# uguryagmur/RealTimeObjectDetection

Measured on AMD Instinct MI355X. Metric: frames/sec YOLOv3 608x608 bs=8 (Darknet.forward + write_results; 2 batches in flight, write_results_async on a second stream), higher is better.
Workload: dtype f16x2-split (3 MFMA products, f32 accumulate); 1 GPU; YOLOv3 cfg 608x608 batch=8 per GPU, split-f16 MFMA conv + fused head + GPU NMS (BASELINE configs[2]); precision=f16s3, tiles=autotune (this run), parallelism=frame-shard x1, in_flight_batches=2, detections_last_step=1699, candidates_last_step=1914, f16_range_overflow=False

## Files before the change

### realtimeobjectdetection_amd/csrc/capi.cpp

```cpp
#include <cstring>
#include <new>

#include "plan.h"

namespace rtod { const std::string& last_error_string(); }
using namespace rtod;

struct rtod_plan { Plan p; };

#define RTOD_GUARD_BEGIN try {
#define RTOD_GUARD_END                                                                   \
    } catch (const std::bad_alloc&) { set_error("out of host memory"); return RTOD_E_ARG; } \
      catch (const std::exception& e) { set_error("internal error: %s", e.what()); return RTOD_E_ARG; } \
      catch (...) { set_error("internal error"); return RTOD_E_ARG; }

extern "C" {

int rtod_version(void) { return 100; }

int rtod_last_error(char* buf, size_t len) {
    if (!buf || !len) return RTOD_E_ARG;
    const std::string& e = last_error_string();
    const size_t n = e.size() < len - 1 ? e.size() : len - 1;
    memcpy(buf, e.data(), n);
// ... 51 lines not shown
    memset(o, 0, sizeof(*o));
    o->n_layers = (int32_t)p.layers.size(); o->n_launches = (int32_t)p.launches.size();
    o->height = p.height; o->width = p.width; o->max_batch = p.max_batch;
    o->total_rows = p.total_rows; o->attrs = p.attrs;
    o->n_weight_floats = p.n_weight_floats; o->conv_flops_per_frame = p.conv_flops;
    o->arena_bytes = p.arena_floats * 4; o->packed_weight_bytes = p.packed_floats * 4;
    return RTOD_OK;
}

int rtod_plan_get_launch(const rtod_plan* plan, int index, rtod_launch_info* out) {
    if (!plan || !out || index < 0 || index >= (int)plan->p.launches.size()) { set_error("plan_get_launch: bad index"); return RTOD_E_ARG; }
    plan->p.fill_launch_info(index, out, plan->p.tuned.empty() ? plan->p.max_batch : plan->p.tuned.rbegin()->first);
    return RTOD_OK;
}

int rtod_plan_describe(const rtod_plan* plan, char* buf, size_t len, size_t* needed) {
    RTOD_GUARD_BEGIN
    if (!plan) { set_error("plan_describe: null plan"); return RTOD_E_ARG; }
    const std::string s = plan->p.describe();
    if (needed) *needed = s.size() + 1;
    if (buf && len) {
        const size_t n = s.size() < len - 1 ? s.size() : len - 1;
        memcpy(buf, s.data(), n);
        buf[n] = 0;
    }
    return RTOD_OK;
    RTOD_GUARD_END
}

const char* rtod_conv_variant_name(int variant) {
    if (variant == 100 + STEM2_VARIANT) return "conv_stem2_f16s3<2 x 4x16, stem + 3x3 s2 + 1x1>";
    if (variant >= 100 + PATCH_VARIANT_BASE && variant < 100 + PATCH_VARIANT_BASE + PATCH_MODES) return conv_patch_mode_info(variant - 100 - PATCH_VARIANT_BASE).name;
    if (variant >= 100 + PWD_VARIANT_BASE && variant < 100 + PWD_VARIANT_BASE + PWD_MODES) return conv_pwd_mode_info(variant - 100 - PWD_VARIANT_BASE).name;
    if (variant >= 100 + RING_VARIANT_BASE && variant < 100 + RING_VARIANT_BASE + RING_MODES) return conv_ring_mode_info(variant - 100 - RING_VARIANT_BASE).name;
    if (variant >= 100 + BAND_VARIANT_BASE && variant < 100 + BAND_VARIANT_BASE + BAND_MODES) return conv_band_mode_info(variant - 100 - BAND_VARIANT_BASE).name;
    if (variant >= 100 && variant < 100 + HV_COUNT) return conv_f16s3_variant_info(variant - 100).name;
    if (variant < 0 || variant % 10 >= CV_COUNT || variant / 10 > 2) return "";
    static const char* const kSliced[2][CV_COUNT] = {
        {"conv_igemm_f32<128x128,w64x64,k-slices>", "conv_igemm_f32<128x64,w64x32,k-slices>", "conv_igemm_f32<64x64,w32x32,k-slices>", "conv_igemm_f32<128x32,w32x32,k-slices>"},
        {"conv_igemm_f32<128x128,w64x64,wg per k-slice>", "conv_igemm_f32<128x64,w64x32,wg per k-slice>", "conv_igemm_f32<64x64,w32x32,wg per k-slice>", "conv_igemm_f32<128x32,w32x32,wg per k-slice>"}};
    if (variant >= 10) return kSliced[variant / 10 - 1][variant % 10];
    return conv_variant_info(variant).name;
}

int rtod_conv_kernel_name(int variant, int epilogue, char* buf, size_t len) {
    if (!buf || len == 0) { set_error("conv_kernel_name: null buffer"); return RTOD_E_ARG; }
    int n = -1;
    if (variant >= 100 + PATCH_VARIANT_BASE) n = conv_patch_kernel_name(variant - 100 - PATCH_VARIANT_BASE, epilogue, buf, len);
    else if (variant >= 100 + PWD_VARIANT_BASE) n = conv_pwd_kernel_name(variant - 100 - PWD_VARIANT_BASE, epilogue, buf, len);
    else if (variant >= 100 + RING_VARIANT_BASE) n = conv_ring_kernel_name(variant - 100 - RING_VARIANT_BASE, epilogue, buf, len);
    else if (variant >= 100 + BAND_VARIANT_BASE) n = conv_band_kernel_name(variant - 100 - BAND_VARIANT_BASE, epilogue, buf, len);
    else if (variant >= 100) n = conv_f16s3_kernel_name(variant - 100, epilogue, buf, len);
    else n = conv_f32_kernel_name(variant, buf, len);
    if (n < 0 || (size_t)n >= len) { set_error("conv_kernel_name: unknown variant %d or buffer too small", variant); return RTOD_E_ARG; }
    return RTOD_OK;
}

int rtod_plan_launch_kernel_name(const rtod_plan* plan, int index, char* buf, size_t len) {
    RTOD_GUARD_BEGIN
    if (!plan || !buf || len == 0 || index < 0 || index >= (int)plan->p.launches.size()) { set_error("launch_kernel_name: bad args"); return RTOD_E_ARG; }
    rtod_launch_info li;
    plan->p.fill_launch_info(index, &li, plan->p.tuned.empty() ? plan->p.max_batch : plan->p.tuned.rbegin()->first);
    buf[0] = 0;
    if (li.kind != LK_CONV || li.flops_per_frame == 0) return RTOD_OK;
    int epi = li.fused_decode ? 2 : (li.fused_pointwise ? (li.fused_residual ? 4 : 3) : (li.fused_residual ? 1 : 0));
    if (plan->p.precision == 2 && li.variant >= 100) epi |= EPI_F16;
    int n = -1;
    if (li.variant == 100 + STEM2_VARIANT) n = conv_stem2_kernel_name(li.fused_pointwise, buf, len);
    else return rtod_conv_kernel_name(li.variant, epi, buf, len);
    if (n < 0 || (size_t)n >= len) { set_error("launch_kernel_name: buffer too small"); return RTOD_E_ARG; }
    return RTOD_OK;
    RTOD_GUARD_END
}

int rtod_plan_set_precision(rtod_plan* plan, int mode) {
    if (!plan || mode < 0 || mode > 2) { set_error("set_precision: mode must be 0 (fp32), 1 (f16 split) or 2 (plain f16)"); return RTOD_E_ARG; }
    if (plan->p.d_weights) { set_error("set_precision: must be called before rtod_plan_load_weights"); return RTOD_E_STATE; }
    if (mode >= 1) { const int rc = plan->p.check_split_supported(mode); if (rc) return rc; }
    plan->p.precision = mode;
    plan->p.layout_weights();
    return RTOD_OK;
}
// ... 196 lines not shown
```

### realtimeobjectdetection_amd/csrc/plan.cpp

```cpp
#include "plan.h"

#include <algorithm>
#include <cctype>
#include <cmath>
#include <cstdarg>
#include <cstdlib>
#include <cstring>
#include <map>
#include <mutex>
#include <sstream>

namespace rtod {

static thread_local std::string g_err;

void set_error(const char* fmt, ...) {
    char buf[1024];
    va_list ap;
    va_start(ap, fmt);
    vsnprintf(buf, sizeof(buf), fmt, ap);
    va_end(ap);
    g_err = buf;
}
const std::string& last_error_string() { return g_err; }
// ... 240 lines not shown
            prev_is_decoded = true;
            pc = layers[i - 1].cout; ph = layers[i - 1].hout; pw = layers[i - 1].wout;
        } else {
            prev_is_decoded = false;
            pc = L.cout; ph = L.hout; pw = L.wout;
        }
        if (L.type == LT_ROUTE || L.type == LT_SHORTCUT) prev_is_decoded = false;
    }
    total_rows = row_off;
    n_weight_floats = woff;
    if (total_rows == 0) { set_error("cfg: no yolo layer (the reference would return [])"); return RTOD_E_CFG; }
    return RTOD_OK;
}

static int resolve_alias(const std::vector<Layer>& layers, int i) {
    while (layers[i].alias_of >= 0) i = layers[i].alias_of;
    return i;
}

void Plan::reset_planning() {
    for (auto& L : layers) { L.fused_into = -1; L.fused_away = false; L.buf = -1; L.coff = 0; L.alias_of = -1; }
    bufs.clear(); launches.clear(); convs.clear(); input_buf = -1;
    tuned.clear(); tune_cache.clear(); tuning.clear();
}

int Plan::set_option(const char* name, int value) {
    if (!name) { set_error("set_option: null name"); return RTOD_E_ARG; }
    if (d_weights) { set_error("set_option: must be called before rtod_plan_load_weights"); return RTOD_E_STATE; }
    const std::string k(name);
    bool* flag = nullptr; int* num = nullptr;
    if (k == "fuse_pointwise") flag = &opt_fuse_pointwise;
    else if (k == "ring_kernel") flag = &opt_ring_kernel;
    else if (k == "pwd_kernel") flag = &opt_pwd_kernel;
    else if (k == "stem2_kernel") flag = &opt_stem2_kernel;
    else if (k == "k_slices") flag = &opt_k_slices;
    else if (k == "bn_batch_stats") {
        if (value && height != width) { set_error("set_option: bn_batch_stats is not supported on a rectangular plan (%dx%d)", height, width); return RTOD_E_ARG; }
        flag = &opt_bn_batch_stats;
    }
    else if (k == "k_slice_workgroups") flag = &opt_k_slice_workgroups;
    else if (k == "patch_kernel") flag = &opt_patch_kernel;
    else if (k == "stem_kernel") flag = &opt_stem_kernel;
    else if (k == "band_kernel") flag = &opt_band_kernel;
    else if (k == "fuse_shortcut") flag = &opt_fuse_shortcut;
    else if (k == "fuse_decode") flag = &opt_fuse_decode;
    else if (k == "zero_copy_concat") flag = &opt_zero_copy_concat;
    else if (k == "force_f16s3_variant") num = &opt_force_f16s3_variant;
    else if (k == "force_f32_variant") num = &opt_force_f32_variant;
    else { set_error("set_option: unknown option '%s'", name); return RTOD_E_ARG; }
    const bool old_flag = flag ? *flag : false; const int old_num = num ? *num : 0;
    if (flag) *flag = value != 0; else *num = value;
    reset_planning();
    int rc = plan_buffers();
    if (!rc && precision >= 1) rc = check_split_supported(precision);
    if (rc) {
        const std::string msg = last_error_string();
        if (flag) *flag = old_flag; else *num = old_num;
        reset_planning();
        (void)plan_buffers();
        set_error("%s", msg.c_str());
    }
    return rc;
}

int Plan::plan_buffers() {
    const int n = (int)layers.size();
// ... 434 lines not shown
    const PackedConv& pc = convs[l.conv_slot];
    if (pc.split || pc.stem || pc.slice_chunks <= 0) return 0;
    const Layer& L = layers[l.layer];
    const ConvVariantInfo& vi = conv_variant_info(variant);
    const int64_t M = (int64_t)batch * L.hout * L.wout;
    const int64_t tiles = ((M + vi.bm - 1) / vi.bm) * ((L.cout + vi.bn - 1) / vi.bn);
    const int64_t S = (pc.Kpad / 32 + pc.slice_chunks - 1) / pc.slice_chunks;
    return (opt_k_slice_workgroups && d_scratch && tiles < 512 && S * M * pc.Npad <= scratch_floats) ? 2 : 1;
}

static bool variant_has_f16(int v) {
    return (v >= 0 && v < HV_COUNT) || (v >= BAND_VARIANT_BASE + BAND_LDS_MODES && v < BAND_VARIANT_BASE + BAND_MODES) ||
           (v >= PWD_VARIANT_BASE && v < PWD_VARIANT_BASE + PWD_MODES);
}
static bool band_mode_ok(int precision, int mode, const Layer& L) {
    return conv_band_mode_valid(mode, L.cin, L.hin, L.win) && (precision != 2 || mode >= BAND_LDS_MODES);
}
static int band_default_mode(int precision, const Layer& L) {
    if (precision != 2) return conv_band_default_mode(L.cin, L.hin, L.win);
    for (int m = BAND_LDS_MODES; m < BAND_MODES; ++m) if (conv_band_mode_valid(m, L.cin, L.hin, L.win)) return m;
    return BAND_LDS_MODES;
}

int Plan::launch_split_variant(ConvArgs& a, const PackedConv& pc, int v, hipStream_t s) const {
    if (precision == 2 && !variant_has_f16(v)) { set_error("variant %d has no plain-f16 instance", v); return RTOD_E_STATE; }
    if (v >= PATCH_VARIANT_BASE) {
        if (pc.band) { set_error("patch variant requested for a band layer"); return RTOD_E_STATE; }
        return launch_conv_patch_f16s3(a, v - PATCH_VARIANT_BASE, s);
    }
    if (v >= PWD_VARIANT_BASE) {
        if (pc.band) { set_error("pointwise variant requested for a band layer"); return RTOD_E_STATE; }
        return launch_conv_pwd_f16s3(a, v - PWD_VARIANT_BASE, s);
    }
    if (v >= RING_VARIANT_BASE) {
        if (pc.band) { set_error("ring variant requested for a band layer"); return RTOD_E_STATE; }
        return launch_conv_ring_f16s3(a, v - RING_VARIANT_BASE, s);
    }
    if (v >= BAND_VARIANT_BASE) {
        if (v == BAND_VARIANT_BASE + BANDD_WIDE_MODE && !pc.band) return launch_conv_bandd_f16s3(a, v - BAND_VARIANT_BASE - BAND_LDS_MODES, s);
        if (!pc.band) { set_error("band variant requested for a layer without band weights"); return RTOD_E_STATE; }
        return launch_conv_band_f16s3(a, v - BAND_VARIANT_BASE, s);
    }
    return launch_conv_f16s3(a, v, s);
}

int Plan::build_conv_args(const Launch& l, int batch, float* out, ConvArgs& a) const {
    const Layer& L = layers[l.layer];
    const PackedConv& pc = convs[l.conv_slot];
    const View in = view_of(l.in_layer);
    a.in = in.base; a.in_ldc = in.ldc; a.in_coff = in.coff;
    a.B = batch; a.Hi = L.hin; a.Wi = L.win; a.Cin = pc.cin_p;
    a.w = d_weights + pc.w_off; a.bias = d_weights + pc.b_off; a.K = pc.K; a.Kpad = pc.Kpad; a.Npad = pc.Npad;
    a.in_bytes = (unsigned)std::min<int64_t>((int64_t)batch * in.H * in.W * in.ldc * 4, 0xFFFFFFFFll);
    a.w_bytes = (unsigned)std::min<int64_t>((int64_t)pc.Npad * pc.Kpad * 2, 0xFFFFFFFFll);
    if (pc.split) {
        a.w_hi = reinterpret_cast<const _Float16*>(d_weights + pc.w_off);
        a.w_lo = reinterpret_cast<const _Float16*>(d_weights + pc.wl_off);
        a.inv_scale = d_weights + pc.s_off;
        a.f16 = precision == 2 ? 1 : 0;
    }
    a.kh = a.kw = L.size; a.stride = L.stride; a.pad = L.pad;
    a.Ho = L.hout; a.Wo = L.wout; a.Cout = L.cout; a.leaky = L.act;
    a.ovf = overflow_flag;
    if (in.C != pc.cin_p || in.H != L.hin || in.W != L.win) { set_error("forward: layer %d input view mismatch", l.layer); return RTOD_E_STATE; }
    if (l.out_layer == -2) { a.out = out; a.dec = l.dec; a.dec.train = train_decode; }
    else {
        const View o = view_of(l.out_layer);
        if (!o.base || o.C != L.cout || o.H != L.hout || o.W != L.wout) { set_error("forward: layer %d output view mismatch", l.layer); return RTOD_E_STATE; }
        a.out = o.base; a.out_ldc = o.ldc; a.out_coff = o.coff; a.out_split = o.split;
    }
    if (l.in2_layer >= 0) {
        const View r = view_of(l.in2_layer);
        if (!r.base || r.C != L.cout || r.H != L.hout || r.W != L.wout) { set_error("forward: layer %d residual view mismatch", l.layer); return RTOD_E_STATE; }
        a.res = r.base; a.res_ldc = r.ldc; a.res_coff = r.coff;
    }
    if (l.pw_guest >= 0 && pw_active()) {
        const Launch& g = launches[l.pw_guest];
        const Layer& G = layers[g.layer];
        const PackedConv& gc = convs[g.conv_slot];
        const View o = view_of(g.out_layer);
        if (!gc.split || gc.Kpad != L.cout || !o.base || !o.split || o.C != G.cout || o.H != L.hout || o.W != L.wout) { set_error("forward: layer %d fused pointwise mismatch", g.layer); return RTOD_E_STATE; }
        a.pw_wh = reinterpret_cast<const _Float16*>(d_weights + gc.w_off);
        a.pw_wl = reinterpret_cast<const _Float16*>(d_weights + gc.wl_off);
        a.pw_inv_scale = d_weights + gc.s_off; a.pw_bias = d_weights + gc.b_off;
        a.pw_out = o.base; a.pw_out_ldc = o.ldc; a.pw_out_coff = o.coff;
        a.pw_cout = G.cout; a.pw_k = L.cout; a.pw_leaky = G.act; a.pw_npad = gc.Npad;
    }
    return RTOD_OK;
}

static std::mutex g_tune_mutex;
static std::map<std::vector<int>, int> g_tune_memo;

int Plan::tune_launch(size_t li, ConvArgs& a, int batch, hipStream_t s) {
    const Launch& l = launches[li];
    const Layer& L = layers[l.layer];
    const bool pw = a.pw_wh != nullptr;
    const std::vector<int> key = {L.cin, L.cout, L.size, L.stride, L.hout, L.wout, l.in2_layer >= 0, l.out_layer == -2, pw ? a.pw_cout : 0,
                                  convs[l.conv_slot].band ? 1 : 0, opt_ring_kernel ? 1 : 0, opt_patch_kernel ? 1 : 0, opt_pwd_kernel ? 1 : 0, L.act,
                                  precision, L.hin, L.win, L.pad};
    auto it = tune_cache.find(key);
    if (it != tune_cache.end()) { tuning[li] = it->second; return RTOD_OK; }
    std::vector<int> gkey = key; gkey.push_back(device); gkey.push_back(batch);
    {
        std::lock_guard<std::mutex> lock(g_tune_mutex);
        auto git = g_tune_memo.find(gkey);
        if (git != g_tune_memo.end()) { tuning[li] = git->second; tune_cache[key] = git->second; return RTOD_OK; }
    }
    hipEvent_t e0, e1;
    RTOD_HIP(hipEventCreate(&e0)); RTOD_HIP(hipEventCreate(&e1));
    std::vector<int> cand;
    if (convs[l.conv_slot].band) {
        for (int m = 0; m < BAND_MODES; ++m) if (band_mode_ok(precision, m, L)) cand.push_back(BAND_VARIANT_BASE + m);
    } else {
        for (int v = 0; v < HV_COUNT; ++v) {
            const ConvVariantInfo& vi = conv_f16s3_variant_info(v);
            if (vi.bn > 2 * ((L.cout + 63) / 64 * 64) && vi.bn > 64) continue;
            if (pw && vi.bn < L.cout) continue;
            cand.push_back(v);
        }
        if (precision == 1 && !pw && L.act <= 1 && opt_patch_kernel && conv_patch_supported(L.size, L.stride, L.pad, L.cin, L.cout) && L.hout == L.hin && l.out_layer != -2)
            for (int m = 0; m < PATCH_MODES; ++m) {
                if (conv_patch_mode_info(m).bn > L.cout && conv_patch_mode_info(m).bn > 64) continue;
                if (!conv_patch_mode_valid(m, L.cin, L.cout)) continue;
                cand.push_back(PATCH_VARIANT_BASE + m);
            }
        if (bandd_wide_candidate(l, L)) cand.push_back(BAND_VARIANT_BASE + BANDD_WIDE_MODE);
        if (pwd_candidate(l, L))
            for (int m = 0; m < PWD_MODES; ++m) {
                if (conv_pwd_mode_info(m).bn > 128 && conv_pwd_mode_info(m).bn > (L.cout + 127) / 128 * 128) continue;
                cand.push_back(PWD_VARIANT_BASE + m);
            }
        if (precision == 1 && !pw && L.act <= 1 && opt_ring_kernel)
            for (int m = 0; m < RING_MODES; ++m) {
                const ConvVariantInfo& vi = conv_ring_mode_info(m);
                if (vi.bn > 2 * ((L.cout + 63) / 64 * 64) && vi.bn > 64) continue;
                cand.push_back(RING_VARIANT_BASE + m);
            }
    }
    int best_v = variant_for(l, batch);
    int rc = RTOD_OK;
    auto time_variant = [&](int v, int reps, int per, float& out_ms) -> int {
        out_ms = 1e30f;
        for (int rep = 0; rep < reps; ++rep) {
            (void)hipEventRecord(e0, s);
            for (int r = 0; r < per; ++r) { const int q = launch_split_variant(a, convs[l.conv_slot], v, s); if (q) return q; }
            (void)hipEventRecord(e1, s);
            if (hipEventSynchronize(e1) != hipSuccess) return hip_fail(hipGetLastError(), "autotune sync");
            float ms = 0.f; (void)hipEventElapsedTime(&ms, e0, e1);
            out_ms = std::min(out_ms, ms / per);
        }
        return RTOD_OK;
    };
    std::vector<std::pair<float, int>> ranked;
    for (int v : cand) {
        rc = launch_split_variant(a, convs[l.conv_slot], v, s);
        if (rc) break;
        float ms; rc = time_variant(v, 3, 2, ms);
        if (rc) break;
        ranked.push_back({ms, v});
    }
    if (!rc && !ranked.empty()) {
        std::sort(ranked.begin(), ranked.end());
        const size_t top = std::min<size_t>(3, ranked.size());
        std::vector<float> fin(top, 1e30f);
        for (int round = 0; round < 5 && !rc; ++round)
            for (size_t t = 0; t < top && !rc; ++t) {
                float ms; rc = time_variant(ranked[t].second, 2, 4, ms);
                fin[t] = std::min(fin[t], ms);
            }
        if (!rc) best_v = ranked[std::min_element(fin.begin(), fin.end()) - fin.begin()].second;
    }
    (void)hipEventDestroy(e0); (void)hipEventDestroy(e1);
    if (rc) return rc;
    tuning[li] = best_v;
    tune_cache[key] = best_v;
    { std::lock_guard<std::mutex> lock(g_tune_mutex); g_tune_memo[gkey] = best_v; }
    return RTOD_OK;
}

int Plan::set_tiles(int batch, const int* variants, int count) {
    if (!variants || count != (int)launches.size() || batch <= 0 || batch > max_batch) { set_error("set_tiles: %d entries for %d launches, batch %d", count, (int)launches.size(), batch); return RTOD_E_ARG; }
    if (precision < 1) { set_error("set_tiles: split-f16 / f16 plans only"); return RTOD_E_STATE; }
    for (int i = 0; i < count; ++i) {
        const int v = variants[i];
        const Launch& l = launches[i];
        if (v < 0) continue;
        if (l.kind != LK_CONV || l.conv_slot < 0 || !convs[l.conv_slot].split) { set_error("set_tiles: launch %d is not a split-f16 convolution", i); return RTOD_E_ARG; }
        const Layer& L = layers[l.layer];
        const bool band = convs[l.conv_slot].band, hosts_pw = l.pw_guest >= 0 && pw_active();
        bool ok;
        if (precision == 2 && !variant_has_f16(v)) ok = false;
        else if (band) ok = v >= BAND_VARIANT_BASE && v < BAND_VARIANT_BASE + BAND_MODES && band_mode_ok(precision, v - BAND_VARIANT_BASE, L);
        else if (v >= PATCH_VARIANT_BASE) ok = v < PATCH_VARIANT_BASE + PATCH_MODES && !hosts_pw && l.out_layer != -2 && L.act <= 1 && L.hout == L.hin &&
                                               conv_patch_supported(L.size, L.stride, L.pad, L.cin, L.cout) && conv_patch_mode_valid(v - PATCH_VARIANT_BASE, L.cin, L.cout);
        else if (v >= PWD_VARIANT_BASE) ok = v < PWD_VARIANT_BASE + PWD_MODES && pwd_candidate(l, L);
        else if (v == BAND_VARIANT_BASE + BANDD_WIDE_MODE) ok = bandd_wide_candidate(l, L);
        else if (v >= RING_VARIANT_BASE) ok = v < RING_VARIANT_BASE + RING_MODES && !hosts_pw && L.act <= 1;
        else ok = v < HV_COUNT && !(hosts_pw && conv_f16s3_variant_info(v).bn < L.cout);
        if (!ok) { set_error("set_tiles: variant %d is not a valid tile of launch %d (layer %d)", v, i, l.layer); return RTOD_E_ARG; }
    }
    tuned[batch] = std::vector<int>(variants, variants + count);
    return RTOD_OK;
}

int Plan::variant_for(const Launch& l, int batch) const {
    const bool band = convs[l.conv_slot].band;
    if (opt_force_f16s3_variant >= 0) {
        const int v = opt_force_f16s3_variant;
        const Layer& FL = layers[l.layer];
        if (band) return band_mode_ok(precision, v - BAND_VARIANT_BASE, FL) ? v : BAND_VARIANT_BASE + band_default_mode(precision, FL);
        if (v == BAND_VARIANT_BASE + BANDD_WIDE_MODE) { if (bandd_wide_candidate(l, FL)) return v; }
        else if (v >= PWD_VARIANT_BASE && v < PWD_VARIANT_BASE + PWD_MODES) { if (pwd_candidate(l, FL)) return v; }
        else if (precision == 1 && v >= RING_VARIANT_BASE && v < RING_VARIANT_BASE + RING_MODES && !(l.pw_guest >= 0 && pw_active()) && FL.act <= 1) return v;
        if (precision == 1 && v >= PATCH_VARIANT_BASE && v < PATCH_VARIANT_BASE + PATCH_MODES && !(l.pw_guest >= 0 && pw_active()) && l.out_layer != -2 && FL.act <= 1 &&
            conv_patch_supported(FL.size, FL.stride, FL.pad, FL.cin, FL.cout) && FL.hout == FL.hin && conv_patch_mode_valid(v - PATCH_VARIANT_BASE, FL.cin, FL.cout)) return v;
        const int g = choose_variant_f16s3(layers[l.layer], batch);
        if (l.pw_guest >= 0 && pw_active() && conv_f16s3_variant_info(g).bn < layers[l.layer].cout) return HV_128x128_8W;
        return g;
    }
    auto it = tuned.find(batch);
    const size_t idx = &l - &launches[0];
    if (it != tuned.end() && idx < it->second.size() && it->second[idx] >= 0) return it->second[idx];
    if (band) return BAND_VARIANT_BASE + band_default_mode(precision, layers[l.layer]);
    const int v = choose_variant_f16s3(layers[l.layer], batch);
    if (l.pw_guest >= 0 && pw_active() && conv_f16s3_variant_info(v).bn < layers[l.layer].cout) return HV_128x128_8W;
    return v;
}

bool Plan::pw_active() const { return precision == 1 && opt_fuse_pointwise; }
bool Plan::bandd_wide_candidate(const Launch& l, const Layer& L) const {
    if (!opt_band_kernel || l.conv_slot < 0 || convs[l.conv_slot].band || !convs[l.conv_slot].split) return false;
    if (l.out_layer == -2 || (l.pw_guest >= 0 && pw_active())) return false;
    const PackedConv& pc = convs[l.conv_slot];
    return conv_bandd_wide_supported(L.size, L.stride, L.pad, pc.cin_p, L.win) && L.hout == L.hin && L.wout == L.win && pc.Npad % 128 == 0 && pc.K == pc.Kpad;
}
bool Plan::pwd_candidate(const Launch& l, const Layer& L) const {
    if (!opt_pwd_kernel || l.conv_slot < 0 || convs[l.conv_slot].band || !convs[l.conv_slot].split) return false;
    if (l.out_layer == -2 || (l.pw_guest >= 0 && pw_active())) return false;
    return conv_pwd_supported(L.size, L.stride, L.pad, convs[l.conv_slot].cin_p) && L.hout == L.hin && L.wout == L.win;
}
bool Plan::stem2_active() const { return precision == 1 && opt_stem2_kernel && stem2_pattern && !keep_all && convs[launches[0].conv_slot].split; }

int Plan::choose_variant_f16s3(const Layer& L, int batch) const {
    if (opt_force_f16s3_variant >= 0 && opt_force_f16s3_variant < HV_COUNT) return opt_force_f16s3_variant;
    if (L.cout <= 64) return HV_128x64;
    const int64_t M = (int64_t)batch * L.hout * L.wout;
    const int64_t gn = (L.cout + 127) / 128;
    if (((M + 127) / 128) * gn >= 512) return HV_128x128;
    if (((M + 63) / 64) * gn >= 512) return HV_64x128;
    return HV_64x64;
}

int Plan::forward(const float* x, int batch, float* out, hipStream_t s, float* launch_ms, bool tune) {
    if (!weights_loaded) { set_error("forward: load_weights has not been called"); return RTOD_E_STATE; }
    if (!x || !out) { set_error("forward: null pointer"); return RTOD_E_ARG; }
    if (batch < 1 || batch > max_batch) { set_error("forward: batch %d outside 1..%d", batch, max_batch); return RTOD_E_ARG; }
    RTOD_HIP(hipSetDevice(device));
    const bool tune_now = tune && precision >= 1 && opt_force_f16s3_variant < 0;
    if (tune_now) { tuning.assign(launches.size(), -1); tune_cache.clear(); }
    const size_t nl = launches.size();
    if (launch_ms && events.size() < 2 * nl) {
        while (events.size() < 2 * nl) { hipEvent_t e; RTOD_HIP(hipEventCreate(&e)); events.push_back(e); }
    }
    for (size_t li = 0; li < nl; ++li) {
        const Launch& l = launches[li];
        if (launch_ms) RTOD_HIP(hipEventRecord(events[2 * li], s));
        int rc = RTOD_OK;
        switch (l.kind) {
            case LK_PACK: {
                View v = view_of(-1);
                rc = launch_pack_input(x, batch, 3, height, width, v.base, 4, s);
                break;
// ... 156 lines not shown
```

### realtimeobjectdetection_amd/csrc/plan.h

```cpp
#pragma once
#include <map>
#include <string>
#include <vector>

#include "rtod_internal.h"

namespace rtod {

enum LayerType { LT_CONV = 0, LT_SHORTCUT, LT_ROUTE, LT_UPSAMPLE, LT_MAXPOOL, LT_YOLO };
const char* layer_type_name(int t);

struct Layer {
    int index = 0;
    int type = LT_CONV;
    int cin = 0, cout = 0, hin = 0, win = 0, hout = 0, wout = 0;
    int size = 0, stride = 1, pad = 0;
    bool bn = false, leaky = false;
    int act = 0;
    bool nearest = false;
    bool decode_v5 = false;
    int pool_pad = 0;
    std::vector<int> srcs;
    std::vector<std::pair<int, int>> anchors;
    int classes = 0, row_offset = 0, rows = 0;
// ... 41 lines not shown
struct Plan {
    int height = 0, width = 0, max_batch = 0, device = 0;
    std::map<std::string, std::string> net_info;
    std::vector<Layer> layers;
    std::vector<Buffer> bufs;
    int input_buf = -1;
    std::vector<Launch> launches;
    std::vector<PackedConv> convs;
    int total_rows = 0, attrs = 0;
    int64_t n_weight_floats = 0, conv_flops = 0;
    int64_t arena_floats = 0, packed_floats = 0;
    float* d_arena = nullptr;
    float* d_weights = nullptr;
    double* d_bn_stats = nullptr;
    int64_t bn_stats_doubles = 0;
    double* d_bn_partial = nullptr;
    int64_t bn_partial_count = 0;
    float* d_scratch = nullptr;
    int64_t scratch_floats = 0;
    bool weights_loaded = false;
    int train_decode = 0;
    int precision = 0;
    bool keep_all = false;
    bool opt_fuse_pointwise = true;
    bool opt_stem_kernel = true;
    bool opt_band_kernel = true;
    bool opt_bn_batch_stats = false;
    bool opt_k_slices = true;
    bool opt_k_slice_workgroups = true;
    bool opt_stem2_kernel = true;
    bool opt_patch_kernel = true;
    bool opt_ring_kernel = true;
    bool opt_pwd_kernel = true;
    bool opt_fuse_shortcut = true;
    bool opt_fuse_decode = true;
    bool opt_zero_copy_concat = true;
    int opt_force_f16s3_variant = -1;
    int opt_force_f32_variant = -1;
    int32_t* overflow_flag = nullptr;
    std::vector<hipEvent_t> events;

    ~Plan();
    int parse(const std::string& cfg_text);
    int resolve_shapes();
    int plan_buffers();
    void assign_arena();
    void layout_weights();
    bool uses_split(const Layer& L, int cin_p) const;
    int check_split_supported(int mode) const;
    int load_weights(const float* w, size_t n);
    int forward(const float* x, int batch, float* out, hipStream_t s, float* launch_ms, bool tune = false);
    int set_option(const char* name, int value);
    int set_tiles(int batch, const int* variants, int count);
    void reset_planning();
    View view_of(int layer) const;
    int choose_variant(const Layer& L, int batch) const;
    int choose_variant_f16s3(const Layer& L, int batch) const;
    int build_conv_args(const Launch& l, int batch, float* out, ConvArgs& a) const;
    int tune_launch(size_t li, ConvArgs& a, int batch, hipStream_t s);
    std::vector<int> tuning;
    std::map<std::vector<int>, int> tune_cache;
    int launch_split_variant(ConvArgs& a, const PackedConv& pc, int v, hipStream_t s) const;
    int variant_for(const Launch& l, int batch) const;
    int f32_slice_mode(const Launch& l, int batch, int variant) const;
    bool pw_active() const;
    bool pwd_candidate(const Launch& l, const Layer& L) const;
    bool bandd_wide_candidate(const Launch& l, const Layer& L) const;
    bool stem2_pattern = false;
    bool stem2_active() const;
    std::map<int, std::vector<int>> tuned;
    std::string describe() const;
    void fill_launch_info(int idx, rtod_launch_info* o, int batch) const;
};

}
```

### realtimeobjectdetection_amd/csrc/rtod_internal.h

```cpp
#pragma once
#include <hip/hip_runtime.h>
#if defined(RTOD_STAMPS) && !defined(RTOD_DIAG)
#define RTOD_DIAG 1
#endif
#include <algorithm>
#include <atomic>
#include <cstdint>
#include <cstdio>
#include <string>
#include <vector>

#include "../../include/rtod.h"

namespace rtod {

void set_error(const char* fmt, ...);
int hip_fail(hipError_t e, const char* what);

#define RTOD_HIP(expr)                                              \
    do {                                                            \
        hipError_t _e = (expr);                                     \
        if (_e != hipSuccess) return ::rtod::hip_fail(_e, #expr);   \
    } while (0)

// ... 116 lines not shown
const ConvVariantInfo& conv_f16s3_variant_info(int v);
int conv_f16s3_kernel_name(int variant, int epi, char* buf, size_t len);
int launch_conv_f16s3(const ConvArgs& a, int variant, hipStream_t s);
bool conv_band_supported(int ksize, int stride, int pad, int cin, int w_in);
constexpr int BANDD_MODES = 9;
constexpr int BAND_LDS_MODES = 11;
constexpr int BAND_MODES = BAND_LDS_MODES + BANDD_MODES;
static_assert(50 + BAND_MODES <= 70, "band variant ids end where the ring kernel's begin");
constexpr int BAND_K2_MODE0 = 7;
const ConvVariantInfo& conv_bandd_mode_info(int idx);
int conv_bandd_mode_kg(int idx);
constexpr int BANDD_WIDE_MODE = BAND_LDS_MODES + 7;
bool conv_bandd_wide_supported(int ksize, int stride, int pad, int cin, int w_in);
int conv_bandd_kernel_name(int idx, int epi, char* buf, size_t len);
int launch_conv_bandd_f16s3(const ConvArgs& a, int idx, hipStream_t s);
int conv_band_layer_kg(int cin, int h, int w);
bool conv_band_mode_valid(int mode, int cin, int h, int w);
int conv_band_default_mode(int cin, int h, int w);
const ConvVariantInfo& conv_band_mode_info(int mode);
int conv_band_kernel_name(int mode, int epi, char* buf, size_t len);
int launch_conv_band_f16s3(const ConvArgs& a, int mode, hipStream_t s);
constexpr int BAND_VARIANT_BASE = 50;
constexpr int RING_MODES = 8;
constexpr int RING_VARIANT_BASE = 70;
const ConvVariantInfo& conv_ring_mode_info(int mode);
int conv_ring_kernel_name(int mode, int epi, char* buf, size_t len);
int launch_conv_ring_f16s3(const ConvArgs& a, int mode, hipStream_t s);
constexpr int PWD_MODES = 11;
constexpr int PWD_VARIANT_BASE = 90;
bool conv_pwd_supported(int ksize, int stride, int pad, int cin);
const ConvVariantInfo& conv_pwd_mode_info(int mode);
int conv_pwd_kernel_name(int mode, int epi, char* buf, size_t len);
int launch_conv_pwd_f16s3(const ConvArgs& a, int mode, hipStream_t s);
constexpr int STEM2_VARIANT = 130;
bool conv_stem2_supported(int k0, int s0, int p0, int cin0, int cout0, int k1, int s1, int p1, int cout1, int pw_cout);
int conv_stem2_kernel_name(int pw, char* buf, size_t len);
int launch_conv_stem2_f16s3(const float* x, int B, int H, int W, const _Float16* w0h, const _Float16* w0l, const float* inv0, const float* bias0,
                            int leaky0, const ConvArgs& c1, hipStream_t s);
constexpr int PATCH_MODES = 5;
constexpr int PATCH_WRES_MODE = 4;
bool conv_patch_mode_valid(int mode, int cin, int cout);
constexpr int PATCH_VARIANT_BASE = 110;
bool conv_patch_supported(int ksize, int stride, int pad, int cin, int cout);
const ConvVariantInfo& conv_patch_mode_info(int mode);
int conv_patch_kernel_name(int mode, int epi, char* buf, size_t len);
int launch_conv_patch_f16s3(const ConvArgs& a, int mode, hipStream_t s);

int launch_conv_stem(const float* x_nchw, const float* w, const float* bias, const View& out, int B, int H, int W,
                     int Ho, int Wo, int stride, int Cout, int leaky, hipStream_t s);
int launch_conv_stem_split(const float* x_nchw, const _Float16* wh, const _Float16* wl, const float* inv_scale, const float* bias,
                           const View& out, int B, int H, int W, int Ho, int Wo, int stride, int Cout, int leaky, int32_t* ovf, hipStream_t s);
int launch_prep_image(const unsigned char* img, int h, int w, int bgr, int inp_dim, float* out, hipStream_t s);
int launch_prep_frames(const unsigned char* frames, int batch, int h, int w, int bgr, int out_h, int out_w, float* out, hipStream_t s);
int launch_pack_input(const float* x_nchw, int B, int C, int H, int W, float* out_nhwc, int Cp, hipStream_t s);
int launch_upsample2x(const View& in, const View& out, int B, hipStream_t s);
int launch_add(const View& a, const View& b, const View& out, int B, hipStream_t s);
int launch_maxpool(const View& in, const View& out, int B, int size, int stride, int pad, hipStream_t s);
int launch_upsample_nearest2x(const View& in, const View& out, int B, hipStream_t s);
int launch_bn_batch(const View& x, const View& y, const View* res, int B, double* stats, int sstride, const float* bn, int gstride, int act,
                    double* partial, int64_t partial_doubles, hipStream_t s);
size_t bn_partial_doubles(int max_channels);
struct BnUpdateEntry { float* running_mean; float* running_var; int64_t stats_off; double unbias; int sstride; int channels; };
constexpr int BN_UPDATE_MAX = 32;
struct BnUpdateTable { BnUpdateEntry e[BN_UPDATE_MAX]; };
int launch_bn_update_running(const BnUpdateEntry* entries, int n, const double* stats, double momentum, hipStream_t s);
int launch_copy(const View& in, const View& out, int B, hipStream_t s);
// ... 14 lines not shown
```

Before: 2536 frames/s.

## Add dedicated stride-2 3x3 split-f16 conv kernel with LDS-DMA stage ring

Adds a new specialised implicit-GEMM kernel for 3x3 stride-2 pad-1 convolutions in split-f16 precision. Per-row tap validity masks and base offsets are precomputed once, then each tap's input is streamed into an LDS ring through buffer-to-LDS DMA with counted vmcnt waits, optionally prefetching across stages. Seven tile modes are registered as autotune candidates for the downsampling layers, enabled by default. This adds code size and tuning time, and the new modes win only where they beat the existing generic tiles.

Result: no change. 2541 frames/s (median of 4 runs) (+0.2%).

```diff
diff --git a/realtimeobjectdetection_amd/csrc/capi.cpp b/realtimeobjectdetection_amd/csrc/capi.cpp
--- a/realtimeobjectdetection_amd/csrc/capi.cpp
+++ b/realtimeobjectdetection_amd/csrc/capi.cpp
@@ -107,6 +107,7 @@
     if (variant == 100 + STEM2_VARIANT) return "conv_stem2_f16s3<2 x 4x16, stem + 3x3 s2 + 1x1>";
     if (variant >= 100 + PATCH_VARIANT_BASE && variant < 100 + PATCH_VARIANT_BASE + PATCH_MODES) return conv_patch_mode_info(variant - 100 - PATCH_VARIANT_BASE).name;
     if (variant >= 100 + PWD_VARIANT_BASE && variant < 100 + PWD_VARIANT_BASE + PWD_MODES) return conv_pwd_mode_info(variant - 100 - PWD_VARIANT_BASE).name;
+    if (variant >= 100 + S2D_VARIANT_BASE && variant < 100 + S2D_VARIANT_BASE + S2D_MODES) return conv_s2d_mode_info(variant - 100 - S2D_VARIANT_BASE).name;
     if (variant >= 100 + RING_VARIANT_BASE && variant < 100 + RING_VARIANT_BASE + RING_MODES) return conv_ring_mode_info(variant - 100 - RING_VARIANT_BASE).name;
     if (variant >= 100 + BAND_VARIANT_BASE && variant < 100 + BAND_VARIANT_BASE + BAND_MODES) return conv_band_mode_info(variant - 100 - BAND_VARIANT_BASE).name;
     if (variant >= 100 && variant < 100 + HV_COUNT) return conv_f16s3_variant_info(variant - 100).name;
@@ -123,6 +124,7 @@
     int n = -1;
     if (variant >= 100 + PATCH_VARIANT_BASE) n = conv_patch_kernel_name(variant - 100 - PATCH_VARIANT_BASE, epilogue, buf, len);
     else if (variant >= 100 + PWD_VARIANT_BASE) n = conv_pwd_kernel_name(variant - 100 - PWD_VARIANT_BASE, epilogue, buf, len);
+    else if (variant >= 100 + S2D_VARIANT_BASE) n = conv_s2d_kernel_name(variant - 100 - S2D_VARIANT_BASE, epilogue, buf, len);
     else if (variant >= 100 + RING_VARIANT_BASE) n = conv_ring_kernel_name(variant - 100 - RING_VARIANT_BASE, epilogue, buf, len);
     else if (variant >= 100 + BAND_VARIANT_BASE) n = conv_band_kernel_name(variant - 100 - BAND_VARIANT_BASE, epilogue, buf, len);
     else if (variant >= 100) n = conv_f16s3_kernel_name(variant - 100, epilogue, buf, len);
diff --git a/realtimeobjectdetection_amd/csrc/conv_s2d_f16s3.hip b/realtimeobjectdetection_amd/csrc/conv_s2d_f16s3.hip
--- /dev/null
+++ b/realtimeobjectdetection_amd/csrc/conv_s2d_f16s3.hip
@@ -0,0 +1,245 @@
+#include "conv_bandd_common.h"
+
+namespace rtod {
+
+template <int BM, int G, int NST, int MINW, int EPI, int XP>
+__global__ __launch_bounds__(256, MINW)
+void conv_s2d_f16s3_kernel(const ConvArgs a, const int grid_m, const int grid_n) {
+    static_assert(EPI == EPI_SPLIT, "plain split-format epilogue only");
+    constexpr int NW = 4, BN = NW * 32, NT = NW * 64, TM = BM / 16, TN = 2;
+    constexpr int LB = 4, LP = 2;
+    constexpr int NBLK = BM / 16;
+    constexpr int NPP = (NBLK + NW - 1) / NW;
+    constexpr int TAPB = BM * 128;
+    constexpr int STAGE = G * TAPB;
+    constexpr int SPC = 9 / G;
+    constexpr int D = LP * G * NPP;
+    static_assert(BM % 16 == 0 && (G == 1 || G == 3) && NST >= 2 && NST <= 4 && G * (NST - 1) >= 2, "stage ring");
+    constexpr int WAIT_STAGE = G * (NST - 1) * LB + (NST - 2) * D;
+    constexpr int WAIT_STAGE_PRO = 2 * LB + (NST - 2) * D;
+    static_assert(WAIT_STAGE >= WAIT_STAGE_PRO && WAIT_STAGE <= 63 && 2 * LB + 2 * D <= 63, "counted waits");
+    constexpr int WAIT_STAGE_XP = G * (NST - 2) * LB + (NST - 3) * D;
+    static_assert(!XP || (NST >= 3 && WAIT_STAGE_XP <= 2 * LB + (NST - 3) * D), "cross-stage prefetch");
+    constexpr int RG = BM * BN * 4 <= 32768 ? BM : (BM / 2) * BN * 4 <= 32768 ? BM / 2 : BM / 4;
+
+    extern __shared__ __attribute__((aligned(16))) unsigned char smem[];
+    const int nwg = grid_m * grid_n;
+    int bid = blockIdx.x;
+    if (!a.xcd_by_n) bid = xcd_remap(bid, nwg);
+    const int bm = bid / grid_n, bn = bid - bm * grid_n;
+    const int tid = (int)threadIdx.x;
+    const int wave = __builtin_amdgcn_readfirstlane(tid >> 6), lane = tid & 63;
+    const int lr = lane & 15, lh = lane >> 4;
+    const int M = a.B * a.Ho * a.Wo;
+    const int m0 = bm * BM;
+    const int PS = (int)a.in_ldc * 4;
+    const unsigned lo_plane = (unsigned)a.in_ldc * 2u;
+
+    const __amdgpu_buffer_rsrc_t rs_a = buffer_rsrc(a.in, a.in_bytes);
+    const __amdgpu_buffer_rsrc_t rs_wh = buffer_rsrc(a.w_hi, a.w_bytes);
+    const __amdgpu_buffer_rsrc_t rs_wl = buffer_rsrc(a.w_lo, a.w_bytes);
+    const unsigned lds0 = (unsigned)(size_t)smem;
+    const int n_cc = a.Cin / 32;
+
+    unsigned dma_vo[NPP], dma_vm[NPP];
+    {
+        const int lrow = lane >> 2;
+        const unsigned cpart = (unsigned)(a.in_coff + (((lane & 3) ^ ((lrow >> 1) & 3)) << 3)) * 2u;
+        const int hw = a.Ho * a.Wo;
+#pragma unroll
+        for (int k = 0; k < NPP; ++k) {
+            const int blk = wave + k * NW;
+            const int m = m0 + blk * 16 + lrow;
+            const bool ok = blk < NBLK && m < M;
+            const int mm = ok ? m : 0;
+            const int b = mm / hw, r = mm - b * hw;
+            const int oy = r / a.Wo, ox = r - oy * a.Wo;
+            const unsigned xm = (ox >= 1 ? 1u : 0u) | 2u | (2 * ox + 1 < a.Wi ? 4u : 0u);
+            const unsigned vm = (oy >= 1 ? xm : 0u) | (xm << 3) | (2 * oy + 1 < a.Hi ? xm << 6 : 0u);
+            dma_vm[k] = ok ? vm : 0u;
+            dma_vo[k] = (unsigned)((b * a.Hi + 2 * oy) * a.Wi + 2 * ox) * (unsigned)PS + cpart;
+        }
+    }
+    auto dma_stage = [&](int cc, auto part_c, int slot) __attribute__((always_inline)) {
+        constexpr int part = decltype(part_c)::value;
+        const bool live = cc < n_cc;
+        const unsigned soff = (unsigned)cc * 64u;
+        const unsigned base = lds0 + (unsigned)(slot * STAGE);
+#pragma unroll
+        for (int k = 0; k < NPP; ++k) asm volatile("" : "+v"(dma_vo[k]), "+v"(dma_vm[k]));
+#pragma unroll
+        for (int g = 0; g < G; ++g) {
+            const int tap = part * G + g;
+            const int toff = ((tap / 3 - 1) * a.Wi + (tap % 3 - 1)) * PS;
+#pragma unroll
+            for (int k = 0; k < NPP; ++k) {
+                const int blk = wave + k * NW;
+                const bool in = live && ((dma_vm[k] >> tap) & 1u);
+                const unsigned vo = in ? dma_vo[k] + (unsigned)toff : OOB;
+                const unsigned dst = blk < NBLK ? base + (unsigned)(g * TAPB + blk * 2048) : lds0 + (unsigned)(NST * STAGE);
+                lds_dma_pair<0x400>(rs_a, vo, soff, lo_plane + soff, dst);
+            }
+        }
+    };
+    const int wn = wave;
+    const int n0 = bn * BN + wn * 32;
+    const unsigned bvoff = n0 + lr < a.Npad ? (unsigned)((n0 + lr) * 32 + lh * 8) * 2u : OOB;
+    const unsigned wchunk = (unsigned)a.Npad * (HBK * 2);
+    const int nsteps = 9 * n_cc;
+    u32x4 Bq[3][TN][2];
+    auto load_b = [&](int t, u32x4 (&q)[TN][2]) __attribute__((always_inline)) {
+        const unsigned vo = t < nsteps ? bvoff : OOB;
+        const unsigned koff = (unsigned)t * wchunk;
+        q[0][0] = buffer_load_b128(rs_wh, vo, koff);
+        q[0][1] = buffer_load_b128(rs_wl, vo, koff);
+        q[1][0] = buffer_load_b128<1024>(rs_wh, vo, koff);
+        q[1][1] = buffer_load_b128<1024>(rs_wl, vo, koff);
+    };
+
+    f32x4 acc[TM][TN];
+#pragma unroll
+    for (int i = 0; i < TM; ++i)
+#pragma unroll
+        for (int j = 0; j < TN; ++j)
+#pragma unroll
+            for (int e = 0; e < 4; ++e) acc[i][j][e] = 0.f;
+
+    typedef const f16x8 __attribute__((address_space(3))) lds_f16x8;
+    int xa = (int)lds0 + lr * 64 + ((lh ^ ((lr >> 1) & 3)) << 4);
+    f16x8 Ah[3], Al[3];
+    auto read_unit = [&](int u, int slotoff, f16x8& h, f16x8& l) __attribute__((always_inline)) {
+        const int o = xa + slotoff;
+        h = *reinterpret_cast<lds_f16x8*>((unsigned)(o + (u / TM) * TAPB + (u % TM) * 2048));
+        l = *reinterpret_cast<lds_f16x8*>((unsigned)(o + (u / TM) * TAPB + (u % TM) * 2048 + 1024));
+    };
+
+    static_assert(NST - 1 <= SPC, "prologue stages lie in chunk 0");
+    dma_stage(0, std::integral_constant<int, 0>{}, 0);
+    if constexpr (NST >= 3) dma_stage(0, std::integral_constant<int, 1>{}, 1);
+    if constexpr (NST >= 4) dma_stage(0, std::integral_constant<int, 2>{}, 2);
+    load_b(0, Bq[0]);
+    load_b(1, Bq[1]);
+
+    __builtin_amdgcn_s_setprio(2);
+    int rs = 0;
+    auto stage_body = [&](int cc, auto part_c) __attribute__((always_inline)) {
+        constexpr int part = decltype(part_c)::value;
+        constexpr int npart = (part + NST - 1) % SPC, ncc = (part + NST - 1) / SPC;
+        if constexpr (XP) vmcnt<WAIT_STAGE_XP>();
+        else if (cc * SPC + part < NST - 1) vmcnt<WAIT_STAGE_PRO>(); else vmcnt<WAIT_STAGE>();
+        __builtin_amdgcn_sched_barrier(0);
+        __builtin_amdgcn_s_barrier();
+        dma_stage(cc + ncc, std::integral_constant<int, npart>{}, rs == 0 ? NST - 1 : rs - 1);
+        const int slotoff = rs * STAGE;
+        rs = rs + 1 == NST ? 0 : rs + 1;
+        const int nextoff = rs * STAGE;
+        constexpr int U0 = XP ? (part * G * TM) % 3 : 0;
+        if (!XP || (part == 0 && cc == 0)) {
+            read_unit(0, slotoff, Ah[U0], Al[U0]);
+            read_unit(1, slotoff, Ah[(U0 + 1) % 3], Al[(U0 + 1) % 3]);
+        }
+        __builtin_amdgcn_sched_barrier(0);
+#pragma unroll
+        for (int u = 0; u < G * TM; ++u) {
+            const int g = u / TM, i = u % TM;
+            const int tap = part * G + g;
+            if (i == 0) {
+                load_b(cc * 9 + tap + 2, Bq[(tap + 2) % 3]);
+                const int n = (tap == 0 ? (G == 1 && cc > 0 ? 1 : 0) : ((tap - 1) % G == 0 ? 1 : 0)) + (tap % G == 0 ? 1 : 0);
+                if (n == 2) vmcnt<2 * LB + 2 * D>(); else if (n == 1) vmcnt<2 * LB + D>(); else vmcnt<2 * LB>();
+                tie_bset<false>(Bq[tap % 3]);
+                __builtin_amdgcn_sched_barrier(0);
+            }
+            if (u + 2 < G * TM) read_unit(u + 2, slotoff, Ah[(U0 + u + 2) % 3], Al[(U0 + u + 2) % 3]);
+            else if constexpr (XP) read_unit(u + 2 - G * TM, nextoff, Ah[(U0 + u + 2) % 3], Al[(U0 + u + 2) % 3]);
+            const f16x8 ah = Ah[(U0 + u) % 3], al = Al[(U0 + u) % 3];
+#pragma unroll
+            for (int jn = 0; jn < TN; ++jn) {
+                const f16x8 bh = __builtin_bit_cast(f16x8, Bq[tap % 3][jn][0]);
+                const f16x8 bl = __builtin_bit_cast(f16x8, Bq[tap % 3][jn][1]);
+                acc[i][jn] = __builtin_amdgcn_mfma_f32_16x16x32_f16(al, bh, acc[i][jn], 0, 0, 0);
+                acc[i][jn] = __builtin_amdgcn_mfma_f32_16x16x32_f16(ah, bl, acc[i][jn], 0, 0, 0);
+                acc[i][jn] = __builtin_amdgcn_mfma_f32_16x16x32_f16(ah, bh, acc[i][jn], 0, 0, 0);
+            }
+            __builtin_amdgcn_sched_barrier(0);
+        }
+    };
+#pragma unroll 1
+    for (int cc = 0; cc < n_cc; ++cc) {
+        asm volatile("" : "+v"(xa));
+        stage_body(cc, std::integral_constant<int, 0>{});
+        stage_body(cc, std::integral_constant<int, 1>{});
+        stage_body(cc, std::integral_constant<int, 2>{});
+        if constexpr (SPC == 9) {
+            stage_body(cc, std::integral_constant<int, 3>{});
+            stage_body(cc, std::integral_constant<int, 4>{});
+            stage_body(cc, std::integral_constant<int, 5>{});
+            stage_body(cc, std::integral_constant<int, 6>{});
+            stage_body(cc, std::integral_constant<int, 7>{});
+            stage_body(cc, std::integral_constant<int, 8>{});
+        }
+    }
+    vmcnt<0>();
+    tie_bset<false>(Bq[0]); tie_bset<false>(Bq[1]); tie_bset<false>(Bq[2]);
+    __builtin_amdgcn_sched_barrier(0);
+    __builtin_amdgcn_s_setprio(0);
+
+    bandd_epilogue<BM, BN, BM, 32, NT, RG, false, 1, false>(a, acc, smem, bm, bn, tid, 0, wn, lr, lh, M, 0);
+}
+
+template <int BM, int G, int NST, int MINW, int XP>
+static int launch_s2d(const ConvArgs& a, hipStream_t s) {
+    constexpr int BN = 128, NT = 256;
+    constexpr int RG = BM * BN * 4 <= 32768 ? BM : (BM / 2) * BN * 4 <= 32768 ? BM / 2 : BM / 4;
+    const int M = a.B * a.Ho * a.Wo;
+    const int gm = (M + BM - 1) / BM, gn = (a.Cout + BN - 1) / BN;
+    ConvArgs ax = a;
+    ax.xcd_by_n = (gn % 8 == 0 && (int64_t)a.Cout * a.K > (int64_t)M * a.Cin) ? 1 : 0;
+    constexpr int ring_bytes = NST * G * BM * 128 + ((BM / 16) % 4 ? 2048 : 0), epi_bytes = RG * BN * 4;
+    constexpr int lds = ring_bytes > epi_bytes ? ring_bytes : epi_bytes;
+    static_assert(lds <= 160 * 1024, "LDS");
+    auto k_plain = conv_s2d_f16s3_kernel<BM, G, NST, MINW, EPI_SPLIT, XP>;
+    if constexpr (lds > 64 * 1024) {
+        static std::atomic<unsigned long long> attr_done{0};
+        if (int rc = lds_opt_in(attr_done, lds, "conv_s2d_f16s3", k_plain)) return rc;
+    }
+    hipLaunchKernelGGL(k_plain, dim3(gm * gn), dim3(NT), lds, s, ax, gm, gn);
+    return hip_fail(hipGetLastError(), "conv_s2d_f16s3 launch");
+}
+
+#define RTOD_S2D_TILES(X) \
+    X(0, 128, 1, 3, 3, 0) X(1, 96, 1, 3, 3, 0) X(2, 64, 3, 2, 3, 0) X(3, 64, 1, 4, 4, 0) X(4, 128, 1, 3, 3, 1) X(5, 96, 1, 3, 3, 1) X(6, 64, 1, 4, 4, 1)
+
+#define RTOD_X_INFO(idx, bm, g, nst, minw, xp) {bm, 128, "conv_s2d_f16s3<" #bm "x128,g" #g ",r" #nst ",xp" #xp ">"},
+static const ConvVariantInfo kS2dModes[S2D_MODES] = { RTOD_S2D_TILES(RTOD_X_INFO) };
+#undef RTOD_X_INFO
+const ConvVariantInfo& conv_s2d_mode_info(int idx) { return kS2dModes[idx < 0 || idx >= S2D_MODES ? 0 : idx]; }
+
+bool conv_s2d_supported(int ksize, int stride, int pad, int cin) { return ksize == 3 && stride == 2 && pad == 1 && cin >= 32 && cin % 32 == 0; }
+
+int conv_s2d_kernel_name(int idx, int epi, char* buf, size_t len) {
+#define RTOD_X_NAME(i, bm, g, nst, minw, xp) \
+    if (idx == i) return snprintf(buf, len, "void rtod::conv_s2d_f16s3_kernel<" #bm ", " #g ", " #nst ", " #minw ", %d, " #xp ">(rtod::ConvArgs, int, int)", epi);
+    RTOD_S2D_TILES(RTOD_X_NAME)
+#undef RTOD_X_NAME
+    return -1;
+}
+
+int launch_conv_s2d_f16s3(const ConvArgs& a, int idx, hipStream_t s) {
+    if (int rc = check_split_conv_args(a, "launch_conv_s2d", false)) return rc;
+    if (!conv_s2d_supported(a.kh, a.stride, a.pad, a.Cin) || a.kw != 3 || a.Ho != (a.Hi - 1) / 2 + 1 || a.Wo != (a.Wi - 1) / 2 + 1 ||
+        a.dec.enabled || a.pw_wh || a.res || a.f16) {
+        set_error("launch_conv_s2d: unsupported shape or epilogue (k=%d s=%d pad=%d Cin=%d res=%d f16=%d)", a.kh, a.stride, a.pad, a.Cin, a.res ? 1 : 0, a.f16);
+        return RTOD_E_ARG;
+    }
+    if (a.in_ldc % 8 || a.in_coff % 8 || a.K != a.Kpad || a.K != 9 * a.Cin || a.Npad % 128) { set_error("launch_conv_s2d: bad view / K"); return RTOD_E_ARG; }
+    switch (idx) {
+#define RTOD_X_CASE(i, bm, g, nst, minw, xp) case i: return launch_s2d<bm, g, nst, minw, xp>(a, s);
+        RTOD_S2D_TILES(RTOD_X_CASE)
+#undef RTOD_X_CASE
+    }
+    set_error("launch_conv_s2d: mode %d unsupported", idx);
+    return RTOD_E_ARG;
+}
+
+}
diff --git a/realtimeobjectdetection_amd/csrc/plan.cpp b/realtimeobjectdetection_amd/csrc/plan.cpp
--- a/realtimeobjectdetection_amd/csrc/plan.cpp
+++ b/realtimeobjectdetection_amd/csrc/plan.cpp
@@ -296,6 +296,7 @@
     if (k == "fuse_pointwise") flag = &opt_fuse_pointwise;
     else if (k == "ring_kernel") flag = &opt_ring_kernel;
     else if (k == "pwd_kernel") flag = &opt_pwd_kernel;
+    else if (k == "s2d_kernel") flag = &opt_s2d_kernel;
     else if (k == "stem2_kernel") flag = &opt_stem2_kernel;
     else if (k == "k_slices") flag = &opt_k_slices;
     else if (k == "bn_batch_stats") {
@@ -796,6 +797,10 @@
         if (pc.band) { set_error("pointwise variant requested for a band layer"); return RTOD_E_STATE; }
         return launch_conv_pwd_f16s3(a, v - PWD_VARIANT_BASE, s);
     }
+    if (v >= S2D_VARIANT_BASE) {
+        if (pc.band) { set_error("stride-2 variant requested for a band layer"); return RTOD_E_STATE; }
+        return launch_conv_s2d_f16s3(a, v - S2D_VARIANT_BASE, s);
+    }
     if (v >= RING_VARIANT_BASE) {
         if (pc.band) { set_error("ring variant requested for a band layer"); return RTOD_E_STATE; }
         return launch_conv_ring_f16s3(a, v - RING_VARIANT_BASE, s);
@@ -862,7 +867,7 @@
     const bool pw = a.pw_wh != nullptr;
     const std::vector<int> key = {L.cin, L.cout, L.size, L.stride, L.hout, L.wout, l.in2_layer >= 0, l.out_layer == -2, pw ? a.pw_cout : 0,
                                   convs[l.conv_slot].band ? 1 : 0, opt_ring_kernel ? 1 : 0, opt_patch_kernel ? 1 : 0, opt_pwd_kernel ? 1 : 0, L.act,
-                                  precision, L.hin, L.win, L.pad};
+                                  precision, L.hin, L.win, L.pad, opt_s2d_kernel ? 1 : 0};
     auto it = tune_cache.find(key);
     if (it != tune_cache.end()) { tuning[li] = it->second; return RTOD_OK; }
     std::vector<int> gkey = key; gkey.push_back(device); gkey.push_back(batch);
@@ -895,6 +900,7 @@
                 if (conv_pwd_mode_info(m).bn > 128 && conv_pwd_mode_info(m).bn > (L.cout + 127) / 128 * 128) continue;
                 cand.push_back(PWD_VARIANT_BASE + m);
             }
+        if (s2d_candidate(l, L)) for (int m = 0; m < S2D_MODES; ++m) cand.push_back(S2D_VARIANT_BASE + m);
         if (precision == 1 && !pw && L.act <= 1 && opt_ring_kernel)
             for (int m = 0; m < RING_MODES; ++m) {
                 const ConvVariantInfo& vi = conv_ring_mode_info(m);
@@ -960,6 +966,7 @@
                                                conv_patch_supported(L.size, L.stride, L.pad, L.cin, L.cout) && conv_patch_mode_valid(v - PATCH_VARIANT_BASE, L.cin, L.cout);
         else if (v >= PWD_VARIANT_BASE) ok = v < PWD_VARIANT_BASE + PWD_MODES && pwd_candidate(l, L);
         else if (v == BAND_VARIANT_BASE + BANDD_WIDE_MODE) ok = bandd_wide_candidate(l, L);
+        else if (v >= S2D_VARIANT_BASE) ok = v < S2D_VARIANT_BASE + S2D_MODES && s2d_candidate(l, L);
         else if (v >= RING_VARIANT_BASE) ok = v < RING_VARIANT_BASE + RING_MODES && !hosts_pw && L.act <= 1;
         else ok = v < HV_COUNT && !(hosts_pw && conv_f16s3_variant_info(v).bn < L.cout);
         if (!ok) { set_error("set_tiles: variant %d is not a valid tile of launch %d (layer %d)", v, i, l.layer); return RTOD_E_ARG; }
@@ -976,6 +983,7 @@
         if (band) return band_mode_ok(precision, v - BAND_VARIANT_BASE, FL) ? v : BAND_VARIANT_BASE + band_default_mode(precision, FL);
         if (v == BAND_VARIANT_BASE + BANDD_WIDE_MODE) { if (bandd_wide_candidate(l, FL)) return v; }
         else if (v >= PWD_VARIANT_BASE && v < PWD_VARIANT_BASE + PWD_MODES) { if (pwd_candidate(l, FL)) return v; }
+        else if (v >= S2D_VARIANT_BASE && v < S2D_VARIANT_BASE + S2D_MODES) { if (s2d_candidate(l, FL)) return v; }
         else if (precision == 1 && v >= RING_VARIANT_BASE && v < RING_VARIANT_BASE + RING_MODES && !(l.pw_guest >= 0 && pw_active()) && FL.act <= 1) return v;
         if (precision == 1 && v >= PATCH_VARIANT_BASE && v < PATCH_VARIANT_BASE + PATCH_MODES && !(l.pw_guest >= 0 && pw_active()) && l.out_layer != -2 && FL.act <= 1 &&
             conv_patch_supported(FL.size, FL.stride, FL.pad, FL.cin, FL.cout) && FL.hout == FL.hin && conv_patch_mode_valid(v - PATCH_VARIANT_BASE, FL.cin, FL.cout)) return v;
@@ -1003,6 +1011,13 @@
     if (!opt_pwd_kernel || l.conv_slot < 0 || convs[l.conv_slot].band || !convs[l.conv_slot].split) return false;
     if (l.out_layer == -2 || (l.pw_guest >= 0 && pw_active())) return false;
     return conv_pwd_supported(L.size, L.stride, L.pad, convs[l.conv_slot].cin_p) && L.hout == L.hin && L.wout == L.win;
+}
+bool Plan::s2d_candidate(const Launch& l, const Layer& L) const {
+    if (!opt_s2d_kernel || precision != 1 || l.conv_slot < 0 || convs[l.conv_slot].band || !convs[l.conv_slot].split) return false;
+    if (l.out_layer == -2 || l.in2_layer >= 0 || (l.pw_guest >= 0 && pw_active())) return false;
+    const PackedConv& pc = convs[l.conv_slot];
+    return conv_s2d_supported(L.size, L.stride, L.pad, pc.cin_p) && L.hout == (L.hin - 1) / 2 + 1 && L.wout == (L.win - 1) / 2 + 1 &&
+           L.cout >= 128 && pc.Npad % 128 == 0 && pc.K == pc.Kpad && pc.K == 9 * pc.cin_p;
 }
 bool Plan::stem2_active() const { return precision == 1 && opt_stem2_kernel && stem2_pattern && !keep_all && convs[launches[0].conv_slot].split; }
 
diff --git a/realtimeobjectdetection_amd/csrc/plan.h b/realtimeobjectdetection_amd/csrc/plan.h
--- a/realtimeobjectdetection_amd/csrc/plan.h
+++ b/realtimeobjectdetection_amd/csrc/plan.h
@@ -97,6 +97,7 @@
     bool opt_patch_kernel = true;
     bool opt_ring_kernel = true;
     bool opt_pwd_kernel = true;
+    bool opt_s2d_kernel = true;
     bool opt_fuse_shortcut = true;
     bool opt_fuse_decode = true;
     bool opt_zero_copy_concat = true;
@@ -130,6 +131,7 @@
     int f32_slice_mode(const Launch& l, int batch, int variant) const;
     bool pw_active() const;
     bool pwd_candidate(const Launch& l, const Layer& L) const;
+    bool s2d_candidate(const Launch& l, const Layer& L) const;
     bool bandd_wide_candidate(const Launch& l, const Layer& L) const;
     bool stem2_pattern = false;
     bool stem2_active() const;
diff --git a/realtimeobjectdetection_amd/csrc/rtod_internal.h b/realtimeobjectdetection_amd/csrc/rtod_internal.h
--- a/realtimeobjectdetection_amd/csrc/rtod_internal.h
+++ b/realtimeobjectdetection_amd/csrc/rtod_internal.h
@@ -172,6 +172,13 @@
 const ConvVariantInfo& conv_pwd_mode_info(int mode);
 int conv_pwd_kernel_name(int mode, int epi, char* buf, size_t len);
 int launch_conv_pwd_f16s3(const ConvArgs& a, int mode, hipStream_t s);
+constexpr int S2D_MODES = 7;
+constexpr int S2D_VARIANT_BASE = 80;
+static_assert(RING_VARIANT_BASE + RING_MODES <= S2D_VARIANT_BASE && S2D_VARIANT_BASE + S2D_MODES <= PWD_VARIANT_BASE, "stride-2 variant ids lie between the ring's and the 1x1 slab tiles'");
+bool conv_s2d_supported(int ksize, int stride, int pad, int cin);
+const ConvVariantInfo& conv_s2d_mode_info(int mode);
+int conv_s2d_kernel_name(int mode, int epi, char* buf, size_t len);
+int launch_conv_s2d_f16s3(const ConvArgs& a, int mode, hipStream_t s);
 constexpr int STEM2_VARIANT = 130;
 bool conv_stem2_supported(int k0, int s0, int p0, int cin0, int cout0, int k1, int s1, int p1, int cout1, int pw_cout);
 int conv_stem2_kernel_name(int pw, char* buf, size_t len);
```
